# JoshuaLim007/VoxelEngine

Measured on AMD Instinct MI355X. Metric: Mrays/s primary+1-bounce @1080p, 8k×512×8k brickmap; % HBM roofline, higher is better.
Workload: dtype f32

## Files before the change

### voxelengine_amd/csrc/vxrt_persist2.hpp

```cpp
#pragma once

#include "vxrt_camera.hpp"
#include "vxrt_kernels.hpp"
#include "vxrt_pixel_map.hpp"
#include "vxrt_wave2.hpp"

namespace vxrt {

enum : uint32_t { PX_NONE = 0u, PX_PRIMARY = 1u, PX_SHADOW = 2u, PX_BOUNCE = 3u, PX_BOUNCE2 = 4u };

enum : int { PF_STAGE = 0, PF_TX, PF_ROW, PF_POS_X, PF_POS_Y, PF_POS_Z, PF_COL_X, PF_COL_Y, PF_COL_Z, PF_PCODE, PF_PSTEPS, PF_OCCL,
             PF_SAMPLE, PF_PIXEL_FIELDS };
enum : int { WV_COUNTERS = 0, WV_LIGHT_DX = 4, WV_LIGHT_DY, WV_LIGHT_DZ, WV_LIGHT_IVX, WV_LIGHT_IVY, WV_LIGHT_IVZ, WV_LIGHT_DN,
             WV_LIGHT_STEP_X, WV_LIGHT_STEP_Y, WV_LIGHT_STEP_Z, WV_SHADOW_FROM_END, WV_WORDS = 16 };
#ifndef VXRT_NO_KERNARG_RELOAD
#define VXRT_KERNARG_RELOAD 1
#endif
__device__ __forceinline__ const RenderArgs& kernarg_reload(const RenderArgs& in_registers)
{
#ifdef VXRT_KERNARG_RELOAD
    auto* p = (const __attribute__((address_space(4))) RenderArgs*)__builtin_amdgcn_kernarg_segment_ptr();
    asm volatile("" : "+s"(p));
    return *(const RenderArgs*)p;
#else
    return in_registers;
#endif
}

#ifndef VXRT_PERSIST2_OCC
#define VXRT_PERSIST2_OCC 5
#endif
#ifndef VXRT_QUEUE_GRANULE
#define VXRT_QUEUE_GRANULE 4u
#endif
#ifndef VXRT_SUBROUNDS2
#define VXRT_SUBROUNDS2 3
#endif
#ifndef VXRT_VOTE2_NEXT
#define VXRT_VOTE2_NEXT 2
#endif
#ifndef VXRT_VOTE2_END
#define VXRT_VOTE2_END 1
#endif
#ifndef VXRT_VOTE2_BOX
#define VXRT_VOTE2_BOX 2
#endif
#ifdef VXRT_VOTE2_ABS_BOX
__device__ __forceinline__ bool vote2(int parked, int others, int num, int k)
{
    (void)num;
    return parked >= k || (parked > 0 && others == 0);
}
#else
#define VXRT_VOTE2_ABS_BOX 0
#define VXRT_VOTE2_ABS_END 0
#define VXRT_VOTE2_ABS_NEXT 0
__device__ __forceinline__ bool vote2(int parked, int others, int num, int k)
{
    (void)k;
    return vote_run(parked, others, num);
}
#endif
#define PX_LD_U(f, v) do { if (LDS) v = PX[(f) * 64]; } while (0)
#define PX_ST_U(f, v) do { if (LDS) PX[(f) * 64] = (uint32_t)(v); } while (0)
#define PX_LD_I(f, v) do { if (LDS) v = (int)PX[(f) * 64]; } while (0)
#define PX_LD_F(f, v) do { if (LDS) v = __uint_as_float(PX[(f) * 64]); } while (0)
#define PX_ST_F(f, v) do { if (LDS) PX[(f) * 64] = __float_as_uint(v); } while (0)
#define PX_LD_POS() do { PX_LD_F(PF_POS_X, position.x); PX_LD_F(PF_POS_Y, position.y); PX_LD_F(PF_POS_Z, position.z); } while (0)
#define PX_ST_POS() do { PX_ST_F(PF_POS_X, position.x); PX_ST_F(PF_POS_Y, position.y); PX_ST_F(PF_POS_Z, position.z); } while (0)
#define PX_LD_COL() do { PX_LD_F(PF_COL_X, color.x); PX_LD_F(PF_COL_Y, color.y); PX_LD_F(PF_COL_Z, color.z); } while (0)
#define PX_ST_COL() do { PX_ST_F(PF_COL_X, color.x); PX_ST_F(PF_COL_Y, color.y); PX_ST_F(PF_COL_Z, color.z); } while (0)

template <bool STATS, bool BOUNCE2, bool MULTI, bool WIDE, bool COMMON = false>
__global__ __launch_bounds__(64, VXRT_PERSIST2_OCC) void k_render_persist2(RenderArgs A_kern)
{
    static_assert(!(COMMON && WIDE), "COMMON launches run on ordinary grids");
    using FT = FrameTraits<COMMON>;
    using Tracer = WaveTracerT<WIDE>;
    constexpr bool LDS = true;
    constexpr bool END_SHADOW = !(BOUNCE2 && MULTI) || COMMON;
    __shared__ uint32_t cold_block[(CF_TRACER_FIELDS + PF_PIXEL_FIELDS) * 64 + WV_WORDS];
    const WorldView& W = A_kern.W;
    const int lane = threadIdx.x & 63;
    uint32_t* const PX = &cold_block[CF_TRACER_FIELDS * 64 + lane];
    auto lane_view = [&](const RenderArgs& A, uint32_t v) -> LaneView {
        if (MULTI) {
            const ViewArgs& S = A.views[v];
            return LaneView{S.origin, S.fwd, S.up, S.right, S.frame_number, S.fb, S.color_aov, FT::hit_aov(S.hit_aov)};
        }
        return LaneView{A.origin, A.fwd, A.up, A.right, A.frame_number, A.fb, A.color_aov, FT::hit_aov(A.hit_aov)};
    };

    Tracer T;
    T.init(W, &cold_block[lane]);
    uint32_t stage = PX_NONE;
    uint32_t px_tx = 0, px_row = 0;
    f3 position = mk3(0, 0, 0), color = mk3(0, 0, 0);
    uint32_t pcode = 0;
    int p_steps = 0;
    float occl = 0.0f;
    int sample = 0;
    uint32_t n_primary = 0, n_shadow = 0, n_bounce = 0, n_hits = 0;
    PX_ST_U(PF_STAGE, stage);
    uint32_t* const WV = &cold_block[(CF_TRACER_FIELDS + PF_PIXEL_FIELDS) * 64];
    if (lane < 4)
        WV[WV_COUNTERS + lane] = 0u;
    {
        const f3 lu = A_kern.light_unit;
        const float dd = dot3(lu, lu);
        f3 ld = unit3_ordinary(lu, dd);
        const float ex = ld.x == 0 ? kFltEps : ld.x, ey = ld.y == 0 ? kFltEps : ld.y, ez = ld.z == 0 ? kFltEps : ld.z;
        float lix = rcp_rn(ex), liy = rcp_rn(ey), liz = rcp_rn(ez);
        if (!(ordinary(dd) & ordinary(ex) & ordinary(ey) & ordinary(ez))) {
            ld = unit3(lu);
            lix = 1.0f / (ld.x == 0 ? kFltEps : ld.x);
            liy = 1.0f / (ld.y == 0 ? kFltEps : ld.y);
            liz = 1.0f / (ld.z == 0 ? kFltEps : ld.z);
        }
        const bool light_special = !(fabsf(ld.x) >= kMinFastDir && fabsf(ld.y) >= kMinFastDir && fabsf(ld.z) >= kMinFastDir);
        const bool aov = FT::want_hit_aov(A_kern, MULTI);
        if (lane == 0) {
            WV[WV_LIGHT_DX] = __float_as_uint(ld.x);
            WV[WV_LIGHT_DY] = __float_as_uint(ld.y);
            WV[WV_LIGHT_DZ] = __float_as_uint(ld.z);
            WV[WV_LIGHT_IVX] = __float_as_uint(lix);
            WV[WV_LIGHT_IVY] = __float_as_uint(liy);
            WV[WV_LIGHT_IVZ] = __float_as_uint(liz);
            WV[WV_LIGHT_DN] = (ld.x > 0 ? 0u : 1u) | (ld.y > 0 ? 0u : 2u) | (ld.z > 0 ? 0u : 4u);
            WV[WV_LIGHT_STEP_X] = __float_as_uint(A_kern.light_step.x);
            WV[WV_LIGHT_STEP_Y] = __float_as_uint(A_kern.light_step.y);
            WV[WV_LIGHT_STEP_Z] = __float_as_uint(A_kern.light_step.z);
            WV[WV_SHADOW_FROM_END] = (END_SHADOW && FT::mode(A_kern) == 0 && A_kern.shadow && !light_special && !aov) ? 1u : 0u;
        }
    }

    uint32_t tile = 0, tile_used = 64u, tile_view = 0;
    uint32_t queue_shard = blockIdx.x % kQueueShards;
    bool drained = false;
    unsigned long long dg_iters = 0, dg_walk = 0, dg_drain = 0;
    unsigned int dg_runs[3] = {0, 0, 0}, dg_lanes[3] = {0, 0, 0};
    const unsigned long long dg_t0 = STATS ? wall_clock64() : 0ull;
    unsigned long long dg_next_ticks = 0, dg_park_ticks = 0;
    unsigned long long dg_co_runs = 0, dg_co_starts = 0;
    unsigned long long dg_end_shadow = 0;
#ifdef VXRT_TAIL_DEBUG
    unsigned long long px_t0 = 0;
#endif


    auto store_pixel = [&](const RenderArgs& A, const PixelCoords& pc, const LaneView& V, f3 origin, bool hit, f3 normal, f3 pos, f3 shaded) {
        PixelSink sink{A, pc.out_row, V.fb, V.color_aov};
        const int Wd = (int)A.width, Hd = (int)A.height;
        if (hit) {
            if (FT::mode(A) == 1) {
                f3 dv = pos - origin;
                float dist = sqrtf(dot3(dv, dv));
                const float wrap = (float)(1.0 + 1e-6);
                f3 hp = mk3(fmodf(pos.x / 128.0f, wrap), fmodf(pos.y / 128.0f, wrap), fmodf(pos.z / 128.0f, wrap));
                if (pc.x < (Wd >> 1) && pc.y < (Hd >> 1))
                    sink.put(pc.x, pc.y, normal);
                else if (pc.x >= (Wd >> 1) && pc.y < (Hd >> 1))
                    sink.put(pc.x, pc.y, hp);
                else if (pc.x < (Wd >> 1)) {
                } else
                    sink.put(pc.x, pc.y, mk3(dist * 0.01f, 0, 0));
            } else {
                if (!MULTI && FT::accum(A))
                    shaded = accumulate_color(A, pc.out_row, pc.x, shaded);
                const float tx = shaded.x + 1.0f, ty = shaded.y + 1.0f, tz = shaded.z + 1.0f;
                f3 c = mk3(div_rn(shaded.x, tx, rcp_rn(tx)), div_rn(shaded.y, ty, rcp_rn(ty)), div_rn(shaded.z, tz, rcp_rn(tz)));
                const bool plain = !(((shaded.x == 0.0f) | ordinary(shaded.x)) & ((shaded.y == 0.0f) | ordinary(shaded.y)) &
                                     ((shaded.z == 0.0f) | ordinary(shaded.z)) & ordinary(tx) & ordinary(ty) & ordinary(tz));
                if (__ballot(plain) != 0ull)
                    c = mk3(shaded.x / (shaded.x + 1.0f), shaded.y / (shaded.y + 1.0f), shaded.z / (shaded.z + 1.0f));
                c = mk3(lo(hi(c.x, 0), 1), lo(hi(c.y, 0), 1), lo(hi(c.z, 0), 1));
                sink.put(pc.x, pc.y, c);
            }
        } else {
            sink.put(pc.x, pc.y, shaded);
        }
        if (pc.tx == (A.width >> 1) && pc.ty == (A.height >> 1)) {
            float ten = 10.0f;
            pin(ten);
            sink.put(pc.x, pc.y, mk3(ten, ten, ten));
        }
        if (FT::mode(A) == 1 && pc.x < (Wd >> 1) && pc.y > (Hd >> 1))
            sink.put(pc.x, pc.y, mk3((float)p_steps / 256.0f, 0, 0));
    };

    auto shadow_from_end = [&](Tracer& Tr, const lanemask_t ended) -> lanemask_t {
        if (ended == 0ull)
            return 0ull;
        bool go = false;
        if (lane_test(ended)) {
            if (PX[PF_STAGE * 64] == PX_PRIMARY && WV[WV_SHADOW_FROM_END] != 0u) {
                TraceResult r;
                Tr.result(W, r);
                const f3 at = r.pos;
                const f3 from = at + mk3(__uint_as_float(WV[WV_LIGHT_STEP_X]), __uint_as_float(WV[WV_LIGHT_STEP_Y]),
                                         __uint_as_float(WV[WV_LIGHT_STEP_Z]));
                const f3 s0 = mk3(from.x * W.inv_f, from.y * W.inv_f, from.z * W.inv_f);
                const uint32_t signs = __float_as_uint(s0.x) | __float_as_uint(s0.y) | __float_as_uint(s0.z);
                if ((int32_t)signs >= 0 && s0.x < (float)W.cx && s0.y < (float)W.cy && s0.z < (float)W.cz) {
                    PX[PF_PCODE * 64] = r.ncode;
                    PX[PF_PSTEPS * 64] = (uint32_t)r.steps;
                    PX[PF_POS_X * 64] = __float_as_uint(at.x);
                    PX[PF_POS_Y * 64] = __float_as_uint(at.y);
                    PX[PF_POS_Z * 64] = __float_as_uint(at.z);
                    PX[PF_COL_X * 64] = 0u;
                    PX[PF_COL_Y * 64] = 0u;
                    PX[PF_COL_Z * 64] = 0u;
                    PX[PF_STAGE * 64] = PX_SHADOW;
                    Tr.cold[CF_RAY_CODES * 64] = (uint32_t)kMaxSteps << 7;
                    Tr.cold[CF_START_X * 64] = __float_as_uint(s0.x);
                    Tr.cold[CF_START_Y * 64] = __float_as_uint(s0.y);
                    Tr.cold[CF_START_Z * 64] = __float_as_uint(s0.z);
                    Tr.cold[CF_LAST_CI * 64] = 0xFFFFFFFFu;
                    Tr.cold[CF_TOTAL * 64] = 0u;
                    Tr.d = mk3(__uint_as_float(WV[WV_LIGHT_DX]), __uint_as_float(WV[WV_LIGHT_DY]), __uint_as_float(WV[WV_LIGHT_DZ]));
                    Tr.ivx = __uint_as_float(WV[WV_LIGHT_IVX]);
                    Tr.ivy = __uint_as_float(WV[WV_LIGHT_IVY]);
                    Tr.ivz = __uint_as_float(WV[WV_LIGHT_IVZ]);
                    Tr.dn = WV[WV_LIGHT_DN];
                    Tr.special = false;
                    Tr.st = ST_WALK;
                    go = true;
                }
            }
        }
        const lanemask_t launched = __ballot(go);
        const uint32_t n = (uint32_t)__popcll(launched);
        if (lane == 0) {
            WV[WV_COUNTERS + 1] += n;
            WV[WV_COUNTERS + 3] += n;
        }
        if (STATS)
            dg_end_shadow += n;
        return launched;
    };

    for (;;) {
        const unsigned long long m_walk = __ballot(T.st == ST_WALK);
        const unsigned long long m_box = __ballot(T.st == ST_BOX);
        const unsigned long long m_end = __ballot(waits_for_end(T.st));
        const unsigned long long m_next = __ballot(T.st == ST_DONE);
        if ((m_walk | m_box | m_end | m_next) == 0ull)
            break;
        const int n_walk = __popcll(m_walk), n_box = __popcll(m_box), n_end = __popcll(m_end), n_next = __popcll(m_next);
        if (STATS) {
            dg_iters += 1;
            dg_walk += (unsigned long long)n_walk;
            dg_drain += drained ? 1ull : 0ull;
        }

        int c_walk = n_walk, c_box = n_box, c_end = n_end, c_next = n_next;
        bool dg_end_ran = false, dg_end_restarted = false;
        if (vote2(c_box, c_walk, VXRT_VOTE2_BOX, VXRT_VOTE2_ABS_BOX)) {
            if (STATS) {
                dg_runs[2] += 1u;
                dg_lanes[2] += (unsigned)c_box;
                dg_park_ticks -= wall_clock64();
            }
            T.template phase_box<STATS>(W);
            if (STATS)
                dg_park_ticks += wall_clock64();
            c_box = 0;
            c_walk = __popcll(__ballot(T.st == ST_WALK));
            c_end = __popcll(__ballot(waits_for_end(T.st)));
        }
        if (vote2(c_end, c_walk + c_box, VXRT_VOTE2_END, VXRT_VOTE2_ABS_END)) {
            if (STATS) {
                dg_runs[1] += 1u;
                dg_lanes[1] += (unsigned)c_end;
                dg_park_ticks -= wall_clock64();
            }
            if constexpr (END_SHADOW)
                T.template phase_end_deferred<STATS>(W, shadow_from_end);
            else
                T.template phase_end_deferred<STATS>(W);
            if (STATS)
                dg_park_ticks += wall_clock64();
            c_end = 0;
            c_walk = __popcll(__ballot(T.st == ST_WALK));
            if (STATS) {
                dg_end_ran = true;
                dg_end_restarted = T.pend_m != 0ull;
            }
            c_next = __popcll(__ballot(T.st == ST_DONE));
        }
        if (vote2(c_next, c_walk + c_box + c_end, VXRT_VOTE2_NEXT, VXRT_VOTE2_ABS_NEXT)) {
            if (STATS) {
                dg_runs[0] += 1u;
                dg_lanes[0] += (unsigned)c_next;
                dg_next_ticks -= wall_clock64();
            }
            const RenderArgs& A = kernarg_reload(A_kern);
            const uint32_t ntx = (A.width + 7u) / 8u, nty = (A.launch_rows + 7u) / 8u, ntiles = ntx * nty;
            const f3 L = A.light_dir;
            const f3 sray = A.light_unit;
            PX_LD_U(PF_STAGE, stage);
            PX_LD_U(PF_TX, px_tx);
            PX_LD_U(PF_ROW, px_row);
            bool launch = false;
            bool c_hit = false, c_shadow = false, c_bounce = false;
            f3 l_origin = mk3(0, 0, 0), l_dir = mk3(1, 0, 0);
            int l_max = kMaxSteps;
            if (T.st == ST_DONE && stage != PX_NONE) {
                const LaneView V = lane_view(A, MULTI ? px_row >> 16 : 0u);
                const PixelCoords pc = pixel_coords<COMMON>(A, V.frame_number, px_tx, MULTI ? px_row & 0xFFFFu : px_row);
                const f3 origin = camera_origin<FT>(A, V, pc.x, pc.y);
                TraceResult r;
                T.result(W, r);
                bool finalize = false, do_shade = false, shadowed = false, bounce = false, bounce2 = false;
                if (stage == PX_PRIMARY) {
                    pcode = r.ncode;
                    p_steps = r.steps;
                    position = r.pos;
                    PX_ST_U(PF_PCODE, pcode);
                    PX_ST_U(PF_PSTEPS, p_steps);
                    PX_ST_POS();
                    if (V.hit_aov)
                        V.hit_aov[(size_t)pc.out_row * A.width + (size_t)pc.x] =
                            r.hit ? (long long)r.vx + (long long)W.X * ((long long)r.vy + (long long)W.Y * (long long)r.vz) : -1ll;
                    c_hit = r.hit;
                    if (r.hit) {
                        color = mk3(0, 0, 0);
                        PX_ST_COL();
                    }
                    if (!(r.hit && FT::mode(A) == 0)) {
                        stage = r.hit ? PX_PRIMARY : PX_NONE;
                        finalize = true;
                    } else if (A.shadow) {
                        c_shadow = true;
                        launch = true;
                        l_origin = position + A.light_step;
                        l_dir = sray;
                        l_max = kMaxSteps;
                        stage = PX_SHADOW;
                    } else {
                        do_shade = true;
                    }
                } else if (stage == PX_SHADOW) {
                    shadowed = r.hit;
                    do_shade = true;
                }
                PX_LD_U(PF_PCODE, pcode);
                const f3 pn = normal_decode(pcode);
                const f3 normal = mk3(-pn.x, -pn.y, -pn.z);
                if (do_shade) {
                    const float l_dot = hi(dot3(normal, L), 0) * (float)(shadowed ? 0 : 1);
                    f3 diffuse = A.light_color * l_dot;
                    float up_dot = normal.x * 0.0f + normal.y * 1.0f + normal.z * 0.0f;
                    float t = (float)((double)up_dot * 0.5 + 0.5);
                    color = diffuse + A.ambient * (0.25f + t * (1.0f - 0.25f));
                    if (!shadowed) {
                        PX_LD_POS();
                        const f3 to_hit = position - origin;
                        const float vdd = dot3(to_hit, to_hit);
                        f3 view = unit3_ordinary(to_hit, vdd);
                        if (__ballot(!ordinary(vdd)) != 0ull)
                            view = unit3(to_hit);
                        f3 refl = reflect3(L, normal);
                        float spec = pow32(hi(dot3(view, refl), 0));
                        color.x += spec * A.light_color.x;
                        color.y += spec * A.light_color.y;
                        color.z += spec * A.light_color.z;
                    }
                    PX_ST_COL();
                    stage = PX_PRIMARY;
                    if ((l_dot == 0 || A.bounce_all_hits) && A.bounce_samples > 0) {
                        occl = 0.0f;
                        sample = 0;
                        PX_ST_F(PF_OCCL, occl);
                        PX_ST_U(PF_SAMPLE, sample);
                        bounce = true;
                    } else {
                        finalize = true;
                    }
                } else if (stage == PX_BOUNCE || (BOUNCE2 && stage == PX_BOUNCE2)) {
                    PX_LD_F(PF_OCCL, occl);
                    PX_LD_I(PF_SAMPLE, sample);
                    if (!r.hit)
                        occl += stage == PX_BOUNCE ? 1.0f : 0.5f;
                    bounce2 = BOUNCE2 && stage == PX_BOUNCE && r.hit;
                    if (!bounce2) {
                        sample += 1;
                        if (sample < A.bounce_samples) {
                            bounce = true;
                        } else {
                            occl = div_rn(occl, A.bounce_samples_f, A.inv_bounce_samples);
                            PX_LD_COL();
                            color = color * occl;
                            PX_ST_COL();
                            stage = PX_PRIMARY;
                            finalize = true;
                        }
                    }
                    PX_ST_F(PF_OCCL, occl);
                    PX_ST_U(PF_SAMPLE, sample);
                }
                if (bounce || bounce2) {
                    PX_LD_POS();
                    const uint32_t seed = pc.ty * A.width + pc.tx;
                    const uint32_t si = seed + (uint32_t)sample * 1000u + (V.frame_number + 1u) * 1000u + (bounce2 ? 500u : 0u);
                    const f3 bn = mk3(bounce2 ? -r.normal.x : normal.x, bounce2 ? -r.normal.y : normal.y,
                                      bounce2 ? -r.normal.z : normal.z);
                    const f3 bo = mk3(bounce2 ? r.pos.x : position.x, bounce2 ? r.pos.y : position.y,
                                      bounce2 ? r.pos.z : position.z);
                    float two = 2.0f;
                    pin(two);
                    f3 sd = mk3(random_float(si) * two - 1, random_float(si * 10u) * two - 1, random_float(si * 100u) * two - 1);
                    {
                        const float sdd = dot3(sd, sd);
                        const f3 raw = sd;
                        sd = unit3_ordinary(raw, sdd);
                        if (__ballot(!ordinary(sdd)) != 0ull)
                            sd = unit3(raw);
                    }
                    if (dot3(sd, bn) < 0)
                        sd = reflect3(sd, bn);
                    c_bounce = true;
                    launch = true;
                    l_origin = bo + bn * 0.01f;
                    l_dir = sd;
                    l_max = 8;
                    stage = bounce2 ? PX_BOUNCE2 : PX_BOUNCE;
                }
                if (finalize) {
                    PX_LD_POS();
                    PX_LD_COL();
                    PX_LD_I(PF_PSTEPS, p_steps);
                    const LaneView Vs = lane_view(A, MULTI ? px_row >> 16 : 0u);
                    store_pixel(A, pc, Vs, origin, stage != PX_NONE, normal, position, color);
#ifdef VXRT_TAIL_DEBUG
                    if (STATS && V.color_aov) {
                        float* o = V.color_aov + ((size_t)pc.out_row * A.width + (size_t)pc.x) * 3;
                        o[0] = (float)(px_t0 & 0xFFFFFFull);
                        o[1] = (float)(wall_clock64() & 0xFFFFFFull);
                        o[2] = (float)p_steps;
                    }
#endif
                    stage = PX_NONE;
                }
            }
            bool got = false;
            uint32_t new_tx = 0, new_row = 0;
            unsigned long long want = __ballot(T.st == ST_DONE && stage == PX_NONE);
            while (want != 0ull && !drained) {
                if (tile_used >= 64u) {
                    tile = queue_take(A.tile_counter, ntiles * (MULTI ? A.nviews : 1u), VXRT_QUEUE_GRANULE, queue_shard, lane);
                    if (tile == kQueueDry) {
                        drained = true;
                        break;
                    }
                    tile_used = 0u;
                    if (MULTI) {
                        tile_view = tile / ntiles;
                        tile -= tile_view * ntiles;
                        const ViewArgs& S = A.views[tile_view];
                        if (S.row_order_n)
                            tile = (uint32_t)S.row_order[tile / ntx] * ntx + tile % ntx;
                    } else if (A.tile_order) {
                        tile = A.tile_order[tile];
                    } else if (A.row_order_n) {
                        tile = (uint32_t)A.row_order[tile / ntx] * ntx + tile % ntx;
                    }
                }
                const uint32_t avail = 64u - tile_used;
                const bool wants = ((want >> lane) & 1ull) != 0ull;
                const uint32_t rank = __builtin_amdgcn_mbcnt_hi((uint32_t)(want >> 32), __builtin_amdgcn_mbcnt_lo((uint32_t)want, 0u));
                if (wants && rank < avail) {
                    const uint32_t p = tile_used + rank;
                    new_tx = (tile % ntx) * 8u + (p & 7u);
                    new_row = (tile / ntx) * 8u + (p >> 3);
                    got = pixel_coords<COMMON>(A, MULTI ? A.views[tile_view].frame_number : A.frame_number, new_tx, new_row).live;
                    if (MULTI)
                        new_row |= tile_view << 16;
                }
                const uint32_t asked = (uint32_t)__popcll(want);
                tile_used += asked < avail ? asked : avail;
                want = __ballot(T.st == ST_DONE && stage == PX_NONE && !got);
            }
            if (got) {
                PX_ST_U(PF_TX, new_tx);
                PX_ST_U(PF_ROW, new_row);
                const LaneView V = lane_view(A, MULTI ? new_row >> 16 : 0u);
                const PixelCoords pc = pixel_coords<COMMON>(A, V.frame_number, new_tx, MULTI ? new_row & 0xFFFFu : new_row);
                camera_ray<FT>(A, V, pc.x, pc.y, l_origin, l_dir);
                color = l_dir;
                PX_ST_COL();
                l_max = kMaxSteps;
                launch = true;
                stage = PX_PRIMARY;
#ifdef VXRT_TAIL_DEBUG
                px_t0 = wall_clock64();
#endif
            }
            if (launch)
                T.begin_ray_deferred(W, l_origin, l_dir, l_max);
            T.after_begin_ray_deferred(launch);
            if (STATS) {
                dg_co_runs += dg_end_ran ? 1ull : 0ull;
                dg_co_starts += (dg_end_restarted && __ballot(launch) != 0ull) ? 1ull : 0ull;
            }
            if (drained && T.st == ST_DONE && stage == PX_NONE)
                T.st = ST_IDLE;
            PX_ST_U(PF_STAGE, stage);
            {
                const uint32_t d0 = (uint32_t)__popcll(__ballot(got)), d1 = (uint32_t)__popcll(__ballot(c_shadow)),
                               d2 = (uint32_t)__popcll(__ballot(c_bounce)), d3 = (uint32_t)__popcll(__ballot(c_hit));
                if (lane == 0) {
                    uint32_t* const C = &WV[WV_COUNTERS];
                    C[0] += d0;
                    C[1] += d1;
                    C[2] += d2;
                    C[3] += d3;
                }
            }
            if (STATS)
                dg_next_ticks += wall_clock64();
        }

        T.start_pending(W);
        T.template probe_pairs<VXRT_SUBROUNDS2, STATS>(W);
    }

    if (lane == 0) {
        const uint32_t* const C = &WV[WV_COUNTERS];
        n_primary = C[0];
        n_shadow = C[1];
        n_bounce = C[2];
        n_hits = C[3];
    }
    const unsigned long long s0 = n_primary, s1 = n_shadow, s2 = n_bounce, s3 = n_hits;
    unsigned long long* const stats = A_kern.stats ? stats_row_of<kStatRows, kStatRowStride>(A_kern.stats, blockIdx.x) : nullptr;
    if (lane == 0 && stats) {
        atomicAdd(&stats[kStatPrimary], s0);
        atomicAdd(&stats[kStatShadow], s1);
        atomicAdd(&stats[kStatBounce], s2);
        atomicAdd(&stats[kStatPrimaryHits], s3);
    }
    if (STATS) {
        const unsigned long long p0 = wave_sum(T.cnt.coarse_probes), p1 = wave_sum(T.cnt.brick_entries), p2 = wave_sum(T.cnt.fine_probes);
        const unsigned long long g0 = wave_sum(T.cnt.slack_loads), g1 = wave_sum(T.cnt.stray_loads);
        if (lane == 0 && stats) {
            atomicAdd(&stats[kStatCoarseProbes], p0);
            atomicAdd(&stats[kStatBrickEntries], p1);
            atomicAdd(&stats[kStatFineProbes], p2);
            atomicAdd(&stats[kStatGuardSlack], g0);
            atomicAdd(&stats[kStatGuardStray], g1);
            atomicAdd(&stats[kStatDbgIters], dg_iters);
            atomicAdd(&stats[kStatDbgWalkLanes], dg_walk);
            atomicAdd(&stats[kStatDbgNextRuns], (unsigned long long)dg_runs[0]);
            atomicAdd(&stats[kStatDbgEndRuns], (unsigned long long)dg_runs[1]);
            atomicAdd(&stats[kStatDbgBoxRuns], (unsigned long long)dg_runs[2]);
            atomicAdd(&stats[kStatDbgNextLanes], (unsigned long long)dg_lanes[0]);
            atomicAdd(&stats[kStatDbgEndLanes], (unsigned long long)dg_lanes[1]);
            atomicAdd(&stats[kStatDbgBoxLanes], (unsigned long long)dg_lanes[2]);
            atomicAdd(&stats[kStatDbgLifetime], wall_clock64() - dg_t0);
            atomicAdd(&stats[kStatDbgDrained], dg_drain);
            atomicAdd(&stats[kStatDbgNextTicks], dg_next_ticks);
            atomicAdd(&stats[kStatDbgParkTicks], dg_park_ticks);
            atomicAdd(&stats[kStatDbgCoRuns], dg_co_runs);
            atomicAdd(&stats[kStatDbgCoStarts], dg_co_starts);
            atomicAdd(&stats[kStatDbgEndShadow], dg_end_shadow);
        }
    }
}
#undef PX_LD_U
#undef PX_ST_U
#undef PX_LD_I
#undef PX_LD_F
#undef PX_ST_F
#undef PX_LD_POS
#undef PX_ST_POS
#undef PX_LD_COL
#undef PX_ST_COL

}
```

Before: 9444.

## Precompute per-tile camera rays and first bounce samples into LDS for COMMON launches

For COMMON launches, when a wave claims a new 8x8 tile, each lane computes the camera ray direction and first bounce sample direction for one tile pixel and stores them in LDS. Later pixel refills read these precomputed values instead of running camera_ray and the RNG per pixel. The sample direction is stashed in the pixel fields previously used for primary step count, sample index and occlusion, and tile indices are made wave-uniform with readfirstlane. This uses more LDS and overlaps field storage, which risks incorrect p_steps/sample values if the aliasing is wrong.

```diff
diff --git a/voxelengine_amd/csrc/vxrt_persist2.hpp b/voxelengine_amd/csrc/vxrt_persist2.hpp
--- a/voxelengine_amd/csrc/vxrt_persist2.hpp
+++ b/voxelengine_amd/csrc/vxrt_persist2.hpp
@@ -61,6 +61,26 @@
     return vote_run(parked, others, num);
 }
 #endif
+enum : int { TS_DIR_X = 0, TS_DIR_Y, TS_DIR_Z, TS_SAMPLE_X, TS_SAMPLE_Y, TS_SAMPLE_Z };
+
+template <bool TWICE>
+__device__ __forceinline__ f3 bounce_sample_dir(uint32_t seed, uint32_t frame_number, int sample, bool bounce2)
+{
+    const uint32_t si = seed + (uint32_t)sample * 1000u + (frame_number + 1u) * 1000u + (bounce2 ? 500u : 0u);
+    float two = 2.0f;
+    pin(two);
+    float one = 1.0f;
+    if (TWICE)
+        pin(one);
+    f3 sd = mk3(random_float(si) * two - one, random_float(si * 10u) * two - one, random_float(si * 100u) * two - one);
+    const float sdd = dot3(sd, sd);
+    const f3 raw = sd;
+    sd = unit3_ordinary(raw, sdd);
+    if (__ballot(!ordinary(sdd)) != 0ull)
+        sd = unit3(raw);
+    return sd;
+}
+
 #define PX_LD_U(f, v) do { if (LDS) v = PX[(f) * 64]; } while (0)
 #define PX_ST_U(f, v) do { if (LDS) PX[(f) * 64] = (uint32_t)(v); } while (0)
 #define PX_LD_I(f, v) do { if (LDS) v = (int)PX[(f) * 64]; } while (0)
@@ -79,7 +99,15 @@
     using Tracer = WaveTracerT<WIDE>;
     constexpr bool LDS = true;
     constexpr bool END_SHADOW = !(BOUNCE2 && MULTI) || COMMON;
-    __shared__ uint32_t cold_block[(CF_TRACER_FIELDS + PF_PIXEL_FIELDS) * 64 + WV_WORDS];
+    constexpr bool TILE = COMMON;
+    constexpr int TS_FIELDS = TILE ? 4 : 0;
+    __shared__ uint32_t cold_block[(CF_TRACER_FIELDS + PF_PIXEL_FIELDS) * 64 + WV_WORDS + TS_FIELDS * 64];
+    static_assert(sizeof(cold_block) <= 7680, "six LDS allocation pieces per wave");
+    auto TS = [&](int f, uint32_t p) -> uint32_t& {
+        const int word = f == TS_SAMPLE_Y ? CF_OFF_XZ * 64 : f == TS_SAMPLE_Z ? CF_OFF_Y * 64
+                         : (CF_TRACER_FIELDS + PF_PIXEL_FIELDS) * 64 + WV_WORDS + f * 64;
+        return cold_block[word + p];
+    };
     const WorldView& W = A_kern.W;
     const int lane = threadIdx.x & 63;
     uint32_t* const PX = &cold_block[CF_TRACER_FIELDS * 64 + lane];
@@ -103,6 +131,9 @@
     uint32_t n_primary = 0, n_shadow = 0, n_bounce = 0, n_hits = 0;
     PX_ST_U(PF_STAGE, stage);
     uint32_t* const WV = &cold_block[(CF_TRACER_FIELDS + PF_PIXEL_FIELDS) * 64];
+    uint32_t* const SD_X = &PX[PF_PSTEPS * 64];
+    uint32_t* const SD_Y = &PX[PF_OCCL * 64];
+    uint32_t* const SD_Z = &PX[PF_SAMPLE * 64];
     if (lane < 4)
         WV[WV_COUNTERS + lane] = 0u;
     {
@@ -203,7 +234,8 @@
                 const uint32_t signs = __float_as_uint(s0.x) | __float_as_uint(s0.y) | __float_as_uint(s0.z);
                 if ((int32_t)signs >= 0 && s0.x < (float)W.cx && s0.y < (float)W.cy && s0.z < (float)W.cz) {
                     PX[PF_PCODE * 64] = r.ncode;
-                    PX[PF_PSTEPS * 64] = (uint32_t)r.steps;
+                    if constexpr (!TILE)
+                        PX[PF_PSTEPS * 64] = (uint32_t)r.steps;
                     PX[PF_POS_X * 64] = __float_as_uint(at.x);
                     PX[PF_POS_Y * 64] = __float_as_uint(at.y);
                     PX[PF_POS_Z * 64] = __float_as_uint(at.z);
@@ -312,12 +344,15 @@
                 TraceResult r;
                 T.result(W, r);
                 bool finalize = false, do_shade = false, shadowed = false, bounce = false, bounce2 = false;
+                bool first = false;
+                f3 first_sd = mk3(0, 0, 0);
                 if (stage == PX_PRIMARY) {
                     pcode = r.ncode;
                     p_steps = r.steps;
                     position = r.pos;
                     PX_ST_U(PF_PCODE, pcode);
-                    PX_ST_U(PF_PSTEPS, p_steps);
+                    if constexpr (!TILE)
+                        PX_ST_U(PF_PSTEPS, p_steps);
                     PX_ST_POS();
                     if (V.hit_aov)
                         V.hit_aov[(size_t)pc.out_row * A.width + (size_t)pc.x] =
@@ -369,6 +404,10 @@
                     PX_ST_COL();
                     stage = PX_PRIMARY;
                     if ((l_dot == 0 || A.bounce_all_hits) && A.bounce_samples > 0) {
+                        if constexpr (TILE) {
+                            first = true;
+                            first_sd = mk3(__uint_as_float(*SD_X), __uint_as_float(*SD_Y), __uint_as_float(*SD_Z));
+                        }
                         occl = 0.0f;
                         sample = 0;
                         PX_ST_F(PF_OCCL, occl);
@@ -402,20 +441,20 @@
                 if (bounce || bounce2) {
                     PX_LD_POS();
                     const uint32_t seed = pc.ty * A.width + pc.tx;
-                    const uint32_t si = seed + (uint32_t)sample * 1000u + (V.frame_number + 1u) * 1000u + (bounce2 ? 500u : 0u);
                     const f3 bn = mk3(bounce2 ? -r.normal.x : normal.x, bounce2 ? -r.normal.y : normal.y,
                                       bounce2 ? -r.normal.z : normal.z);
                     const f3 bo = mk3(bounce2 ? r.pos.x : position.x, bounce2 ? r.pos.y : position.y,
                                       bounce2 ? r.pos.z : position.z);
-                    float two = 2.0f;
-                    pin(two);
-                    f3 sd = mk3(random_float(si) * two - 1, random_float(si * 10u) * two - 1, random_float(si * 100u) * two - 1);
-                    {
-                        const float sdd = dot3(sd, sd);
-                        const f3 raw = sd;
-                        sd = unit3_ordinary(raw, sdd);
-                        if (__ballot(!ordinary(sdd)) != 0ull)
-                            sd = unit3(raw);
+                    f3 sd;
+                    if constexpr (TILE) {
+                        sd = first_sd;
+                        if (!first) {
+                            int number;
+                            PX_LD_I(PF_SAMPLE, number);
+                            sd = bounce_sample_dir<true>(seed, V.frame_number, number, bounce2);
+                        }
+                    } else {
+                        sd = bounce_sample_dir<false>(seed, V.frame_number, sample, bounce2);
                     }
                     if (dot3(sd, bn) < 0)
                         sd = reflect3(sd, bn);
@@ -429,7 +468,8 @@
                 if (finalize) {
                     PX_LD_POS();
                     PX_LD_COL();
-                    PX_LD_I(PF_PSTEPS, p_steps);
+                    if constexpr (!TILE)
+                        PX_LD_I(PF_PSTEPS, p_steps);
                     const LaneView Vs = lane_view(A, MULTI ? px_row >> 16 : 0u);
                     store_pixel(A, pc, Vs, origin, stage != PX_NONE, normal, position, color);
 #ifdef VXRT_TAIL_DEBUG
@@ -449,6 +489,8 @@
             while (want != 0ull && !drained) {
                 if (tile_used >= 64u) {
                     tile = queue_take(A.tile_counter, ntiles * (MULTI ? A.nviews : 1u), VXRT_QUEUE_GRANULE, queue_shard, lane);
+                    if constexpr (TILE)
+                        tile = (uint32_t)__builtin_amdgcn_readfirstlane((int)tile);
                     if (tile == kQueueDry) {
                         drained = true;
                         break;
@@ -458,12 +500,40 @@
                         tile_view = tile / ntiles;
                         tile -= tile_view * ntiles;
                         const ViewArgs& S = A.views[tile_view];
-                        if (S.row_order_n)
+                        if constexpr (TILE) {
+                            if (((const __attribute__((address_space(4))) ViewArgs*)&S)->row_order_n)
+                                tile = (uint32_t)__builtin_amdgcn_readfirstlane((int)S.row_order[tile / ntx]) * ntx + tile % ntx;
+                        } else if (S.row_order_n)
                             tile = (uint32_t)S.row_order[tile / ntx] * ntx + tile % ntx;
                     } else if (A.tile_order) {
                         tile = A.tile_order[tile];
                     } else if (A.row_order_n) {
                         tile = (uint32_t)A.row_order[tile / ntx] * ntx + tile % ntx;
+                    }
+                    if constexpr (TILE) {
+                        tile = (uint32_t)__builtin_amdgcn_readfirstlane((int)tile);
+                        const uint32_t ptx = (tile % ntx) * 8u + ((uint32_t)lane & 7u), prow = (tile / ntx) * 8u + ((uint32_t)lane >> 3);
+                        const auto* const S = (const __attribute__((address_space(4))) ViewArgs*)(A.views + (MULTI ? tile_view : 0u));
+                        const uint32_t frame_number = MULTI ? S->frame_number : A.frame_number;
+                        const PixelCoords tp = pixel_coords<COMMON>(A, frame_number, ptx, prow);
+                        LaneView TV{A.origin, A.fwd, A.up, A.right, frame_number, nullptr, nullptr, nullptr};
+                        if (MULTI) {
+                            TV.origin = mk3(S->origin.x, S->origin.y, S->origin.z);
+                            TV.fwd = mk3(S->fwd.x, S->fwd.y, S->fwd.z);
+                            TV.up = mk3(S->up.x, S->up.y, S->up.z);
+                            TV.right = mk3(S->right.x, S->right.y, S->right.z);
+                        }
+                        f3 t_origin, t_dir;
+                        camera_ray<FT>(A, TV, tp.x, tp.y, t_origin, t_dir);
+                        TS(TS_DIR_X, lane) = __float_as_uint(t_dir.x);
+                        TS(TS_DIR_Y, lane) = __float_as_uint(t_dir.y);
+                        TS(TS_DIR_Z, lane) = __float_as_uint(t_dir.z);
+                        if (A.bounce_samples > 0) {
+                            const f3 sd = bounce_sample_dir<true>(tp.ty * A.width + tp.tx, frame_number, 0, false);
+                            TS(TS_SAMPLE_X, lane) = __float_as_uint(sd.x);
+                            TS(TS_SAMPLE_Y, lane) = __float_as_uint(sd.y);
+                            TS(TS_SAMPLE_Z, lane) = __float_as_uint(sd.z);
+                        }
                     }
                 }
                 const uint32_t avail = 64u - tile_used;
@@ -476,17 +546,37 @@
                     got = pixel_coords<COMMON>(A, MULTI ? A.views[tile_view].frame_number : A.frame_number, new_tx, new_row).live;
                     if (MULTI)
                         new_row |= tile_view << 16;
+                    if constexpr (TILE) {
+                        if (got) {
+                            PX_ST_U(PF_TX, new_tx);
+                            PX_ST_U(PF_ROW, new_row);
+                        }
+                        l_dir = mk3(__uint_as_float(TS(TS_DIR_X, p)), __uint_as_float(TS(TS_DIR_Y, p)), __uint_as_float(TS(TS_DIR_Z, p)));
+                        if (A.bounce_samples > 0) {
+                            *SD_X = TS(TS_SAMPLE_X, p);
+                            *SD_Y = TS(TS_SAMPLE_Y, p);
+                            *SD_Z = TS(TS_SAMPLE_Z, p);
+                        }
+                    }
                 }
                 const uint32_t asked = (uint32_t)__popcll(want);
                 tile_used += asked < avail ? asked : avail;
                 want = __ballot(T.st == ST_DONE && stage == PX_NONE && !got);
             }
             if (got) {
-                PX_ST_U(PF_TX, new_tx);
-                PX_ST_U(PF_ROW, new_row);
+                if constexpr (TILE) {
+                    PX_LD_U(PF_ROW, new_row);
+                } else {
+                    PX_ST_U(PF_TX, new_tx);
+                    PX_ST_U(PF_ROW, new_row);
+                }
                 const LaneView V = lane_view(A, MULTI ? new_row >> 16 : 0u);
-                const PixelCoords pc = pixel_coords<COMMON>(A, V.frame_number, new_tx, MULTI ? new_row & 0xFFFFu : new_row);
-                camera_ray<FT>(A, V, pc.x, pc.y, l_origin, l_dir);
+                if constexpr (TILE) {
+                    l_origin = V.origin;
+                } else {
+                    const PixelCoords pc = pixel_coords<COMMON>(A, V.frame_number, new_tx, MULTI ? new_row & 0xFFFFu : new_row);
+                    camera_ray<FT>(A, V, pc.x, pc.y, l_origin, l_dir);
+                }
                 color = l_dir;
                 PX_ST_COL();
                 l_max = kMaxSteps;
```

New measurement: 9620, median of 4. 1.02x the previous value.
